# LeonardoTemperanza/LupinPathTracer

Measured on AMD Instinct MI355X. Metric: Msamples/sec (paths x bounces), higher is better.
Workload: dtype f32; 1 GPU; bistro_class 3840x2160, 16 bounces, 8 spp per step, Standard integrator, software BVH (BASELINE configs[4] frame; stand-in scene for bistroexterior, SURVEY 8d); frames_in_flight=1, frames_per_wavefront=6, first_pass_stack_entries=26, traversal=binary

## Files before the change

### lupinpathtracer_amd/csrc/lupin_stages.hpp

```cpp
#pragma once

#include <hip/hip_runtime.h>
#include <hip/hip_fp16.h>

#include "lupin_device.hpp"
#include "../../include/lupin_tiles.h"

using namespace lpd;


constexpr uint32_t META_BOUNCE_MASK = 0xFFFu;
constexpr uint32_t META_VOLUME = 1u << 12;
constexpr uint32_t META_NEXT_EMISSION = 1u << 13;
constexpr uint32_t META_TERMINATED = 1u << 14;
constexpr uint32_t META_SAMPLE_SHIFT = 16;
constexpr uint32_t HIT_MISS = 0xFFFFFFFFu;

template <typename T>
struct PathField
{
    char *base;
    uint32_t stride;
    __device__ __forceinline__ T &operator[](size_t slot) const { return *reinterpret_cast<T *>(base + slot * stride); }
};
// ... 97 lines not shown
    ori = mk3(m[0][0] * e.x + m[1][0] * e.y + m[2][0] * e.z + m[3][0] * 1.0f,
              m[0][1] * e.x + m[1][1] * e.y + m[2][1] * e.z + m[3][1] * 1.0f,
              m[0][2] * e.x + m[1][2] * e.y + m[2][2] * e.z + m[3][2] * 1.0f);
    dir = normalize3(mk3(m[0][0] * d.x + m[1][0] * d.y + m[2][0] * d.z + m[3][0] * 0.0f,
                         m[0][1] * d.x + m[1][1] * d.y + m[2][1] * d.z + m[3][1] * 0.0f,
                         m[0][2] * d.x + m[1][2] * d.y + m[2][2] * d.z + m[3][2] * 0.0f));
}

__device__ __forceinline__ void slot_to_pixel(const FrameParams &fp, uint32_t slot, uint32_t &gx, uint32_t &gy)
{
    if (fp.tile_px)
    {
        const uint32_t per_tile = fp.tile_px * fp.tile_px;
        const uint32_t t = lupin_owned_tile(slot / per_tile, fp.rank, fp.world, fp.tiles_x);
        const uint32_t r = slot % per_tile;
        gx = (t % fp.tiles_x) * fp.tile_px + r % fp.tile_px;
        gy = (t / fp.tiles_x) * fp.tile_px + r / fp.tile_px;
        return;
    }
    gx = fp.off_x + slot % fp.reg_w;
    gy = fp.off_y + slot / fp.reg_w;
}

__device__ __forceinline__ void queue_append(bool alive, uint32_t slot, uint32_t *queue, uint32_t *counter)
{
    const unsigned long long mask = __ballot(alive);
    if (mask)
    {
        const int lane = threadIdx.x & 63;
        const int leader = __ffsll((long long)mask) - 1;
        uint32_t base = 0;
        if (lane == leader) base = atomicAdd(counter, (uint32_t)__popcll(mask));
        base = __shfl(base, leader);
        if (alive) queue[base + __popcll(mask & ((1ull << lane) - 1ull))] = slot;
    }
}


__global__ void k_set_params(FrameParams fp, FrameParams *dst) { *dst = fp; }

template <bool ADAPTIVE>
__device__ __forceinline__ void begin_paths(const FrameParams *__restrict__ fpp, PathBuffers pb, uint32_t n,
                                            const uint8_t *__restrict__ block_active, const uint32_t *__restrict__ frames, uint32_t blocks_x)
{
    const FrameParams fp = *fpp;
    uint32_t slot = blockIdx.x * LP_BLOCK + threadIdx.x;
    uint32_t gx = 0, gy = 0, frame = 0;
    bool live = slot < n;
    if (live)
    {
        uint32_t pslot;
        frame = slot_frame(fp, slot, pslot);
        slot_to_pixel(fp, pslot, gx, gy);
        live = gx < fp.width && gy < fp.height;
        if (ADAPTIVE && live) live = block_active[(gy >> 3) * blocks_x + (gx >> 3)] != 0;
    }
    const uint32_t shard = blockIdx.x % LP_SHARDS;
    queue_append(live, slot, pb.queue[0] + (size_t)shard * pb.shard_cap, &pb.counts[shard]);
    if (!live) return;
    const FrameParams &ff = fpp[frame];
    uint32_t counter = ff.pc.accum_counter;
    if (ADAPTIVE) counter += frames[(size_t)gy * fp.width + gx];
    uint32_t rng = rng_seed_for(gy * fp.width + gx, counter);
    f3 o, d;
    camera_ray(ff, gx, gy, rng, o, d);
    pb.ori_rng[slot] = make_float4(o.x, o.y, o.z, __uint_as_float(rng));
    pb.dir_meta[slot] = make_float4(d.x, d.y, d.z, __uint_as_float(META_NEXT_EMISSION));
    pb.weight[slot] = make_float4(1.0f, 1.0f, 1.0f, 0.0f);
    pb.radiance[slot] = make_float4(0.0f, 0.0f, 0.0f, 0.0f);
    pb.color[slot] = make_float4(0.0f, 0.0f, 0.0f, 0.0f);
    pb.next_hit[slot] = make_float4(0.0f, 0.0f, 0.0f, __uint_as_float(HIT_MISS));
    pb.next_tri[slot] = 0u;
}

__global__ void __launch_bounds__(LP_BLOCK) k_begin(const FrameParams *__restrict__ fpp, PathBuffers pb, uint32_t n)
{
    begin_paths<false>(fpp, pb, n, nullptr, nullptr, 0u);
}

#ifndef LP_EXTEND_WAVES
#define LP_EXTEND_WAVES 4
#endif
#ifndef LP_SHADE_WAVES
#define LP_SHADE_WAVES 3
#endif
#ifndef LP_DEFER_SHADE_WAVES
#define LP_DEFER_SHADE_WAVES 4
#endif
#ifndef LP_LIGHT_PDF_WAVES
#define LP_LIGHT_PDF_WAVES 4
#endif
#ifndef LP_LIGHT_PDF_MIS_WAVES
#define LP_LIGHT_PDF_MIS_WAVES 3
#endif
#ifndef LP_MIS_DEFER_SHADE_WAVES
#define LP_MIS_DEFER_SHADE_WAVES 3
#endif
#ifndef LP_SIMPLE_SHADE_WAVES
#define LP_SIMPLE_SHADE_WAVES 4
#endif
#ifndef LP_MIS_SHADE_WAVES
#define LP_MIS_SHADE_WAVES 2
#endif
template <bool LDSGEO> struct GeoOf { typedef GeoGlobal type; };
template <> struct GeoOf<true> { typedef GeoLds type; };
template <bool LDSGEO>
__device__ __forceinline__ typename GeoOf<LDSGEO>::type make_geo(const SceneDev &sc, uint32_t *lds, uint32_t stack_words);
template <>
__device__ __forceinline__ GeoGlobal make_geo<false>(const SceneDev &sc, uint32_t *, uint32_t) { return geo_global(sc); }
template <>
__device__ __forceinline__ GeoLds make_geo<true>(const SceneDev &sc, uint32_t *lds, uint32_t stack_words)
{
    GeoLds g = geo_stage_lds(sc, lds + stack_words);
    __syncthreads();
    return g;
}

template <typename Geo, bool OPAQUE = false>
__device__ __forceinline__ void trace_alpha(const Geo &geo, const SceneDev &sc, uint32_t *stack, f3 o, f3 d, uint32_t &rng, float eps,
                                            float4 &hitrec, uint32_t &hit_tri)
{
    float total = 0.0f;
    Closest c;
    c.t = LP_F32_MAX; c.u = 0.0f; c.v = 0.0f; c.tri = 0u; c.inst = HIT_MISS;
    bool hit = false;
    for (uint32_t k = 0; k < 128u; k++)
    {
        c = scene_closest(geo, sc, stack, o, d, eps);
        hit = (c.t != LP_F32_MAX);
        if (!hit) break;
        total += c.t;
        if (OPAQUE || !(sc.instances[c.inst].flags & 1u)) break;
        Surface s = resolve_surface(sc, c.inst, c.tri, c.u, c.v);
        float opacity = surface_opacity(sc, s);
        if (opacity < 1.0f && rnd(rng) >= opacity) o = add(o, scale(d, c.t));
        else break;
    }
    hitrec = make_float4(total, c.u, c.v, __uint_as_float(hit ? c.inst : HIT_MISS));
    hit_tri = c.tri;
}

constexpr int LP_TALLY = 4;
constexpr int LP_ROUND_BASE = 12, LP_ROUND_WORDS = 10;
constexpr int LP_CLOCK_BASE = 22, LP_CLOCK_WORDS = 6;
__device__ __forceinline__ void tally_flush(const uint32_t (&tally)[LP_TALLY], unsigned long long *work)
{
    #pragma unroll
    for (int k = 0; k < LP_TALLY; k++)
    {
        uint32_t v = tally[k];
        #pragma unroll
        for (int off = 32; off > 0; off >>= 1) v += __shfl_xor(v, off);
        if ((threadIdx.x & 63u) == 0u && v) atomicAdd(&work[k], (unsigned long long)v);
    }
}
template <typename Geo, bool COUNT> struct TallyOf { typedef Geo type; };
template <typename Geo> struct TallyOf<Geo, true> { typedef GeoTally<Geo> type; };
template <bool COUNT, typename Geo>
__device__ __forceinline__ typename TallyOf<Geo, COUNT>::type with_tally(const Geo &geo, uint32_t *tally)
{
    if constexpr (COUNT) { GeoTally<Geo> g; g.base = geo; g.tally = tally; return g; }
    else return geo;
}

template <int TYPE, bool LDSGEO, bool OPAQUE, bool COUNT>
__global__ void __attribute__((amdgpu_waves_per_eu(LP_EXTEND_WAVES, 8))) __launch_bounds__(LP_BLOCK) k_extend(SceneDev sc, const FrameParams *__restrict__ fpp, PathBuffers pb, uint32_t iter,
                                                     unsigned long long *shard_stats, uint32_t stack_words, unsigned long long *work)
// ... 399 lines not shown
    const auto geo = geo_global(sc);
    for (uint32_t k = 0; k < (MODE == 1 ? 2u : 1u); k++)
    {
        bool have = i < count;
        f3 o = splat(0.0f), d = mk3(0.0f, 0.0f, 1.0f);
        if (have)
        {
            const uint32_t slot = pb.queue[iter & 1][(size_t)shard * pb.shard_cap + i];
            if (MODE == 0)
            {
                const float4 orr = pb.ori_rng[slot], dm = pb.dir_meta[slot];
                o = mk3(orr.x, orr.y, orr.z); d = mk3(dm.x, dm.y, dm.z);
            }
            else
            {
                const float4 so = pb.sh_org[slot];
                have = (__float_as_uint(so.w) & (1u << k)) != 0;
                const float4 dd = k ? pb.sh_d1[slot] : pb.sh_d0[slot];
                o = mk3(so.x, so.y, so.z); d = mk3(dd.x, dd.y, dd.z);
            }
        }
        if (have)
        {
            const Closest a = scene_closest(geo, sc, lds_stack, o, d, eps);
            bool flag;
            uint32_t why = 0u;
            const Closest b = scene_closest_wide(geo, sc, lds_stack, wide_pairs, o, d, eps, flag, &why);
            why_tie += (why & WIDE_WHY_TIE) ? 1u : 0u; why_cond += (why & WIDE_WHY_CONDITION) ? 1u : 0u;
            why_leaky += (why & WIDE_WHY_LEAKY) ? 1u : 0u; why_stack += (why & WIDE_WHY_STACK) ? 1u : 0u;
            const bool miss_a = a.t == LP_F32_MAX, miss_b = b.t == LP_F32_MAX;
            const bool same = (miss_a && miss_b) || (!miss_a && !miss_b && __float_as_uint(a.t) == __float_as_uint(b.t) && __float_as_uint(a.u) == __float_as_uint(b.u) &&
                                                     __float_as_uint(a.v) == __float_as_uint(b.v) && a.tri == b.tri && a.inst == b.inst);
            checked += 1u; flagged += flag ? 1u : 0u; raw += same ? 0u : 1u; bad += (!same && !flag) ? 1u : 0u;
            if (!same && !flag)
                printf("[lupin verify] uncertified difference: mode %d o %a %a %a d %a %a %a | binary t %a tri %u inst %u | wide t %a tri %u inst %u\n", MODE,
                       o.x, o.y, o.z, d.x, d.y, d.z, a.t, a.tri, a.inst, b.t, b.tri, b.inst);
        }
    }
    uint32_t v[8] = {checked, flagged, bad, raw, why_tie, why_cond, why_leaky, why_stack};
    #pragma unroll
    for (int k = 0; k < 8; k++)
    {
        uint32_t x = v[k];
        #pragma unroll
        for (int off = 32; off > 0; off >>= 1) x += __shfl_xor(x, off);
        if ((threadIdx.x & 63u) == 0u && x) atomicAdd(&verify[k], (unsigned long long)x);
    }
}

__device__ __forceinline__ f3 clamp_radiance(f3 r, float max_radiance)
{
    if (!finite3(r)) r = splat(0.0f);
    if (r.x > max_radiance || r.y > max_radiance || r.z > max_radiance)
        r = scale(r, max_radiance / maxf(r.x, maxf(r.y, r.z)));
    return r;
}

struct ShadowRays
{
    PathBuffers *pb;
    uint32_t slot;
    uint32_t flags;
    __device__ __forceinline__ void emit(int k, f3 org, f3 dir, f3 factor, float scalar)
    {
        flags |= 1u << k;
        if (!pb) return;
        pb->sh_org[slot] = make_float4(org.x, org.y, org.z, 0.0f);
        if (k == 0) { pb->sh_d0[slot] = make_float4(dir.x, dir.y, dir.z, scalar); pb->sh_f0[slot] = make_float4(factor.x, factor.y, factor.z, 0.0f); }
        else        { pb->sh_d1[slot] = make_float4(dir.x, dir.y, dir.z, scalar); pb->sh_f1[slot] = make_float4(factor.x, factor.y, factor.z, 0.0f); }
    }
};

struct PathRegs
{
    f3 ori, dir, weight, radiance;
    uint32_t rng;
    int bounce;
    bool in_medium;
    bool next_emission;
    Medium medium;
    bool pending;
    f3 pend_f;
    float pend_bp;
};

__device__ __forceinline__ bool weight_checks_and_roulette(PathRegs &p)
{
    if (is_zero3(p.weight) || !finite3(p.weight)) return false;
    if (p.bounce > 3)
    {
        float survive = minf(0.99f, maxf(p.weight.x, maxf(p.weight.y, p.weight.z)));
        if (rnd(p.rng) >= survive) return false;
        p.weight = scale(p.weight, 1.0f / survive);
    }
    return true;
}

template <int TYPE, typename Geo, bool SIMPLE = false, bool DEFER = false>
__device__ __forceinline__ bool integrate_vertex(const Geo &geo, const SceneDev &sc, uint32_t *stack, const FrameParams &fp, PathRegs &p,
                                 float4 hitrec, uint32_t hit_tri, ShadowRays &sh)
{
    static_assert(!DEFER || TYPE == LUPIN_PATHTRACE_STANDARD || TYPE == LUPIN_PATHTRACE_MIS, "the light-pdf stage serves the Standard and MIS integrators");
    constexpr bool DEFER_WEIGHT = DEFER && TYPE == LUPIN_PATHTRACE_STANDARD;
    const float eps = fp.pc.ray_epsilon;
    const uint32_t hit_inst = __float_as_uint(hitrec.w);
    p.pending = false;
    if (hit_inst == HIT_MISS)
    {
        if (TYPE != LUPIN_PATHTRACE_DIRECT || p.next_emission)
            p.radiance = add(p.radiance, mul(p.weight, environment_radiance(sc, p.dir)));
        return false;
    }
    const float hit_dst = hitrec.x;

    bool in_volume = false;
    float volume_dst = hit_dst;
    if (p.in_medium)
    {
        float r1 = rnd(p.rng);
        float r2 = rnd(p.rng);
        volume_dst = medium_sample_distance(p.medium.density, hit_dst, r1, r2);
        f3 tr = medium_transmittance(p.medium.density, volume_dst);
        float tp = medium_distance_pdf(p.medium.density, volume_dst, hit_dst);
        p.weight = mul(p.weight, divs(tr, tp));
        in_volume = volume_dst < hit_dst;
    }

    const f3 outgoing = neg(p.dir);
    f3 incoming = splat(0.0f);
    f3 hit_pos;
    if (!in_volume)
    {
        hit_pos = add(p.ori, scale(p.dir, hit_dst));
        const Surface s = resolve_surface(sc, hit_inst, hit_tri, hitrec.y, hitrec.z);
        const MatPoint mp = material_point<SIMPLE>(sc, s);
        const f3 normal = shading_normal(geo, sc, s);

        if (TYPE == LUPIN_PATHTRACE_STANDARD || TYPE == LUPIN_PATHTRACE_NAIVE || p.next_emission)
            p.radiance = add(p.radiance, mul(p.weight, mp.emission));

        const bool delta = mat_is_delta(mp);

        if (TYPE == LUPIN_PATHTRACE_DIRECT)
        {
            if (!delta)
            {
                f3 li = lights_sample(sc, hit_pos, p.rng);
                float pdf = lights_pdf(geo, sc, stack, hit_pos, li, eps);
                f3 bsdfcos = bsdf_eval(mp, normal, outgoing, li);
                if (none_zero3(bsdfcos) && pdf > 0.0f)
                {
                    sh.emit(1, hit_pos, li, mul(p.weight, bsdfcos), pdf);
                }
                p.next_emission = false;
            }
            else p.next_emission = true;
        }

        if (!delta)
        {
            if (TYPE == LUPIN_PATHTRACE_STANDARD || TYPE == LUPIN_PATHTRACE_DIRECT)
            {
                if (rnd(p.rng) < 0.5f)
                {
                    float rnl = rnd(p.rng);
                    float ra = rnd(p.rng), rb = rnd(p.rng);
                    incoming = bsdf_sample(mp, normal, outgoing, rnl, ra, rb);
                }
                else incoming = lights_sample(sc, hit_pos, p.rng);
                if (is_zero3(incoming)) return false;
                if (DEFER_WEIGHT)
                {
                    p.pend_bp = bsdf_pdf(mp, normal, outgoing, incoming);
                    p.pend_f = bsdf_eval(mp, normal, outgoing, incoming);
                    p.pending = true;
                }
                else
                {
                    float prob = 0.5f * bsdf_pdf(mp, normal, outgoing, incoming) + 0.5f * lights_pdf(geo, sc, stack, hit_pos, incoming, eps);
                    p.weight = mul(p.weight, divs(bsdf_eval(mp, normal, outgoing, incoming), prob));
                }
            }
            else if (TYPE == LUPIN_PATHTRACE_NAIVE)
            {
                float rnl = rnd(p.rng);
                float ra = rnd(p.rng), rb = rnd(p.rng);
                incoming = bsdf_sample(mp, normal, outgoing, rnl, ra, rb);
                if (is_zero3(incoming)) return false;
                p.weight = mul(p.weight, divs(bsdf_eval(mp, normal, outgoing, incoming), bsdf_pdf(mp, normal, outgoing, incoming)));
            }
            else
            {
                f3 bsdfcos0 = splat(0.0f);
                float b_pdf0 = 0.0f;
                bool have0 = false;
                #pragma unroll(DEFER ? 2 : 1)
                for (int k = 0; k < 2; k++)
                {
                    const bool light_turn = (k != 0);
                    f3 normal_k = normal, outgoing_k = outgoing;
                    MatPoint mp_k = mp;
                    asm volatile("" : "+v"(normal_k.x), "+v"(normal_k.y), "+v"(normal_k.z), "+v"(outgoing_k.x), "+v"(outgoing_k.y), "+v"(outgoing_k.z),
                                      "+v"(mp_k.color.x), "+v"(mp_k.color.y), "+v"(mp_k.color.z), "+v"(mp_k.roughness), "+v"(mp_k.metallic), "+v"(mp_k.ior));
                    f3 mi;
                    if (light_turn) mi = lights_sample(sc, hit_pos, p.rng);
                    else
                    {
                        float rnl = rnd(p.rng);
                        float ra = rnd(p.rng), rb = rnd(p.rng);
                        mi = bsdf_sample(mp_k, normal_k, outgoing_k, rnl, ra, rb);
                    }
                    if (is_zero3(mi)) break;
                    if (!light_turn) incoming = mi;

                    if (DEFER)
                    {
                        const f3 bsdfcos = bsdf_eval(mp_k, normal_k, outgoing_k, mi);
                        const float bp = bsdf_pdf(mp_k, normal_k, outgoing_k, mi);
                        if (!light_turn) { bsdfcos0 = bsdfcos; b_pdf0 = bp; have0 = true; }
                        if (none_zero3(bsdfcos)) sh.emit(k, hit_pos, mi, mul(p.weight, bsdfcos), bp);
                        continue;
                    }
                    const float light_pdf = lights_pdf(geo, sc, stack, hit_pos, mi, eps);
                    const f3 bsdfcos = bsdf_eval(mp_k, normal_k, outgoing_k, mi);
                    const float b_pdf = bsdf_pdf(mp_k, normal_k, outgoing_k, mi);
                    if (!light_turn) { bsdfcos0 = bsdfcos; b_pdf0 = b_pdf; have0 = true; }
                    float mis_w;
                    if (light_turn) mis_w = (light_pdf * light_pdf) / (light_pdf * light_pdf + b_pdf * b_pdf) / light_pdf;
                    else            mis_w = (b_pdf * b_pdf) / (b_pdf * b_pdf + light_pdf * light_pdf) / b_pdf;

                    if (none_zero3(bsdfcos) && mis_w != 0.0f) sh.emit(k, hit_pos, mi, mul(p.weight, bsdfcos), mis_w);
                }
                if (have0) p.weight = mul(p.weight, divs(bsdfcos0, b_pdf0));
                else p.weight = mul(p.weight, divs(bsdf_eval(mp, normal, outgoing, incoming), bsdf_pdf(mp, normal, outgoing, incoming)));
                p.next_emission = false;
            }
        }
        else
        {
            incoming = delta_sample(mp, normal, outgoing, rnd(p.rng));
            if (is_zero3(incoming)) return false;
            p.weight = mul(p.weight, divs(delta_eval(mp, normal, outgoing, incoming), delta_pdf(mp, normal, outgoing, incoming)));
            if (TYPE == LUPIN_PATHTRACE_MIS) p.next_emission = true;
        }

        if (mat_is_volumetric(mp) && dot3(normal, outgoing) * dot3(normal, incoming) < 0.0f)
        {
            if (!p.in_medium)
            {
                p.medium.density = mp.density;
                p.medium.scattering = mp.scattering;
                p.medium.anisotropy = mp.anisotropy;
                p.in_medium = true;
            }
            else p.in_medium = false;
        }
    }
    else
    {
        hit_pos = add(p.ori, scale(p.dir, volume_dst));
        if (TYPE == LUPIN_PATHTRACE_NAIVE)
        {
            float unused0 = rnd(p.rng); (void)unused0;
            float ra = rnd(p.rng), rb = rnd(p.rng);
            incoming = phase_sample(p.medium, outgoing, ra, rb);
            if (is_zero3(incoming)) return false;
            float prob = phase_pdf(p.medium, outgoing, incoming);
            p.weight = mul(p.weight, divs(phase_eval(p.medium, outgoing, incoming), prob));
        }
        else
        {
            if (rnd(p.rng) < 0.5f)
            {
                float unused0 = rnd(p.rng); (void)unused0;
                float ra = rnd(p.rng), rb = rnd(p.rng);
                incoming = phase_sample(p.medium, outgoing, ra, rb);
            }
            else incoming = lights_sample(sc, hit_pos, p.rng);
            if (TYPE == LUPIN_PATHTRACE_MIS) p.next_emission = true;
            if (is_zero3(incoming)) return false;
            if (DEFER_WEIGHT)
            {
                p.pend_bp = phase_pdf(p.medium, outgoing, incoming);
                p.pend_f = phase_eval(p.medium, outgoing, incoming);
                p.pending = true;
            }
            else
            {
                float prob = 0.5f * phase_pdf(p.medium, outgoing, incoming) + 0.5f * lights_pdf(geo, sc, stack, hit_pos, incoming, eps);
                p.weight = mul(p.weight, divs(phase_eval(p.medium, outgoing, incoming), prob));
            }
        }
    }

    p.ori = hit_pos;
    p.dir = incoming;
    if (DEFER_WEIGHT && p.pending) return true;
    return weight_checks_and_roulette(p);
}

template <int TYPE>
__device__ __forceinline__ bool path_epilogue(const FrameParams &fp, const FrameParams *fpp, PathBuffers &pb, uint32_t slot, PathRegs &p, uint32_t sample, bool cont,
                                              bool vol_dirty, float4 r4)
{
    bool alive = false;
    if (cont)
    {
        alive = true;
        if (vol_dirty)
        {
            pb.vol0[slot] = make_float4(p.medium.density.x, p.medium.density.y, p.medium.density.z, p.medium.anisotropy);
            pb.vol1[slot] = make_float4(p.medium.scattering.x, p.medium.scattering.y, p.medium.scattering.z, 0.0f);
        }
        pb.weight[slot] = make_float4(p.weight.x, p.weight.y, p.weight.z, 0.0f);
        if (p.radiance.x != r4.x || p.radiance.y != r4.y || p.radiance.z != r4.z)
            pb.radiance[slot] = make_float4(p.radiance.x, p.radiance.y, p.radiance.z, 0.0f);
    }
    else
    {
        float4 c4 = pb.color[slot];
        f3 cr = clamp_radiance(p.radiance, fp.pc.max_radiance);
        pb.color[slot] = make_float4(c4.x + cr.x, c4.y + cr.y, c4.z + cr.z, 0.0f);
        sample++;
        if (sample < fp.spp)
        {
            alive = true;
            uint32_t gx, gy, pslot;
            const uint32_t frame = slot_frame(fp, slot, pslot);
            slot_to_pixel(fp, pslot, gx, gy);
            camera_ray(fpp[frame], gx, gy, p.rng, p.ori, p.dir);
            p.bounce = 0;
            p.in_medium = false;
            p.next_emission = true;
            pb.weight[slot] = make_float4(1.0f, 1.0f, 1.0f, 0.0f);
            pb.radiance[slot] = make_float4(0.0f, 0.0f, 0.0f, 0.0f);
            if (TYPE == LUPIN_PATHTRACE_MIS)
            {
                pb.next_hit[slot] = make_float4(0.0f, 0.0f, 0.0f, __uint_as_float(HIT_MISS));
                pb.next_tri[slot] = 0u;
            }
        }
    }
    if (alive)
    {
        uint32_t nm = ((uint32_t)p.bounce & META_BOUNCE_MASK) | (p.in_medium ? META_VOLUME : 0u) |
                      (p.next_emission ? META_NEXT_EMISSION : 0u) | (sample << META_SAMPLE_SHIFT);
        pb.ori_rng[slot] = make_float4(p.ori.x, p.ori.y, p.ori.z, __uint_as_float(p.rng));
        pb.dir_meta[slot] = make_float4(p.dir.x, p.dir.y, p.dir.z, __uint_as_float(nm));
    }
    return alive;
}

enum : int { SLOT_DONE = 0, SLOT_ALIVE = 1, SLOT_WAITS_FOR_LIGHT_PDF = 2 };
constexpr uint32_t QUEUE_STATE_SHIFT = 30u, QUEUE_SLOT_MASK = (1u << QUEUE_STATE_SHIFT) - 1u, QUEUE_ENTRY_NONE = 0xFFFFFFFFu;

template <int TYPE, typename Geo, bool SIMPLE = false, bool DEFER = false>
__device__ __forceinline__ int shade_path(const Geo &geo, const SceneDev &sc, uint32_t *stack, const FrameParams &fp, const FrameParams *fpp, PathBuffers &pb,
                                          uint32_t slot, float4 orr, float4 dm, uint32_t rng, float4 hitrec, uint32_t hit_tri)
{
    float4 w4 = pb.weight[slot];
    float4 r4 = pb.radiance[slot];
    uint32_t meta = __float_as_uint(dm.w);

    PathRegs p;
    p.ori = mk3(orr.x, orr.y, orr.z);
    p.dir = mk3(dm.x, dm.y, dm.z);
    p.weight = mk3(w4.x, w4.y, w4.z);
    p.radiance = mk3(r4.x, r4.y, r4.z);
    p.rng = rng;
    p.bounce = (int)(meta & META_BOUNCE_MASK);
    p.in_medium = SIMPLE ? false : (meta & META_VOLUME) != 0;
    p.next_emission = (meta & META_NEXT_EMISSION) != 0;
    uint32_t sample = meta >> META_SAMPLE_SHIFT;
    const bool was_in_medium = p.in_medium;
    if (p.in_medium)
    {
        float4 a = pb.vol0[slot], b = pb.vol1[slot];
        p.medium.density = mk3(a.x, a.y, a.z);
        p.medium.anisotropy = a.w;
        p.medium.scattering = mk3(b.x, b.y, b.z);
    }
    else { p.medium.density = splat(0.0f); p.medium.scattering = splat(0.0f); p.medium.anisotropy = 0.0f; }

    ShadowRays sh;
    sh.pb = (TYPE == LUPIN_PATHTRACE_MIS || TYPE == LUPIN_PATHTRACE_DIRECT) ? &pb : nullptr;
    sh.slot = slot;
    sh.flags = 0u;
    bool cont = integrate_vertex<TYPE, Geo, SIMPLE, DEFER>(geo, sc, stack, fp, p, hitrec, hit_tri, sh);
    const bool vol_dirty = p.in_medium && !was_in_medium;
    if (DEFER && cont && p.pending)
    {
        if (vol_dirty)
        {
            pb.vol0[slot] = make_float4(p.medium.density.x, p.medium.density.y, p.medium.density.z, p.medium.anisotropy);
            pb.vol1[slot] = make_float4(p.medium.scattering.x, p.medium.scattering.y, p.medium.scattering.z, 0.0f);
        }
        if (was_in_medium) pb.weight[slot] = make_float4(p.weight.x, p.weight.y, p.weight.z, 0.0f);
        if (p.radiance.x != r4.x || p.radiance.y != r4.y || p.radiance.z != r4.z)
            pb.radiance[slot] = make_float4(p.radiance.x, p.radiance.y, p.radiance.z, 0.0f);
        pb.sh_f0[slot] = make_float4(p.pend_f.x, p.pend_f.y, p.pend_f.z, p.pend_bp);
        const uint32_t nm = ((uint32_t)p.bounce & META_BOUNCE_MASK) | (p.in_medium ? META_VOLUME : 0u) |
                            (p.next_emission ? META_NEXT_EMISSION : 0u) | (sample << META_SAMPLE_SHIFT);
        pb.ori_rng[slot] = make_float4(p.ori.x, p.ori.y, p.ori.z, __uint_as_float(p.rng));
        pb.dir_meta[slot] = make_float4(p.dir.x, p.dir.y, p.dir.z, __uint_as_float(nm));
        return SLOT_WAITS_FOR_LIGHT_PDF;
    }
    if (cont)
    {
        p.bounce++;
        if (p.bounce > (int)fp.max_bounces) cont = false;
    }

    if (TYPE == LUPIN_PATHTRACE_MIS || TYPE == LUPIN_PATHTRACE_DIRECT)
    {
        if (vol_dirty)
        {
            pb.vol0[slot] = make_float4(p.medium.density.x, p.medium.density.y, p.medium.density.z, p.medium.anisotropy);
            pb.vol1[slot] = make_float4(p.medium.scattering.x, p.medium.scattering.y, p.medium.scattering.z, 0.0f);
        }
        pb.weight[slot] = make_float4(p.weight.x, p.weight.y, p.weight.z, 0.0f);
        pb.radiance[slot] = make_float4(p.radiance.x, p.radiance.y, p.radiance.z, 0.0f);
        const uint32_t nm = ((uint32_t)p.bounce & META_BOUNCE_MASK) | (p.in_medium ? META_VOLUME : 0u) |
                            (p.next_emission ? META_NEXT_EMISSION : 0u) | (cont ? 0u : META_TERMINATED) | (sample << META_SAMPLE_SHIFT);
        pb.ori_rng[slot] = make_float4(p.ori.x, p.ori.y, p.ori.z, __uint_as_float(p.rng));
        pb.dir_meta[slot] = make_float4(p.dir.x, p.dir.y, p.dir.z, __uint_as_float(nm));
        pb.sh_org[slot].w = __uint_as_float(sh.flags);
        return SLOT_ALIVE;
    }
    return path_epilogue<TYPE>(fp, fpp, pb, slot, p, sample, cont, vol_dirty, r4) ? SLOT_ALIVE : SLOT_DONE;
}

template <int TYPE, typename Geo>
__device__ __forceinline__ bool light_pdf_path(const Geo &geo, const SceneDev &sc, uint32_t *stack, const FrameParams &fp, const FrameParams *fpp, PathBuffers &pb, uint32_t slot)
{
    const float4 orr = pb.ori_rng[slot], dm = pb.dir_meta[slot], w4 = pb.weight[slot], pd = pb.sh_f0[slot];
    const uint32_t meta = __float_as_uint(dm.w);
    PathRegs p;
    p.ori = mk3(orr.x, orr.y, orr.z);
    p.dir = mk3(dm.x, dm.y, dm.z);
    p.weight = mk3(w4.x, w4.y, w4.z);
    p.rng = __float_as_uint(orr.w);
    p.bounce = (int)(meta & META_BOUNCE_MASK);
    p.in_medium = (meta & META_VOLUME) != 0;
    p.next_emission = (meta & META_NEXT_EMISSION) != 0;
    p.pending = false;
    const uint32_t sample = meta >> META_SAMPLE_SHIFT;

    const float prob = 0.5f * pd.w + 0.5f * lights_pdf(geo, sc, stack, p.ori, p.dir, fp.pc.ray_epsilon);
    p.weight = mul(p.weight, divs(mk3(pd.x, pd.y, pd.z), prob));
    bool cont = weight_checks_and_roulette(p);
    if (cont)
    {
        p.bounce++;
        if (p.bounce > (int)fp.max_bounces) cont = false;
    }
    float4 r4 = make_float4(0.0f, 0.0f, 0.0f, 0.0f);
    if (!cont) r4 = pb.radiance[slot];
    p.radiance = mk3(r4.x, r4.y, r4.z);
    return path_epilogue<TYPE>(fp, fpp, pb, slot, p, sample, cont, false, r4);
}

#ifndef LP_SORT_WINDOW
#define LP_SORT_WINDOW 4096
#endif
template <bool PEEK_COIN, bool FROM_TRACER>
__global__ void __launch_bounds__(LP_BLOCK) k_sort_queue(SceneDev sc, PathBuffers pb, uint32_t iter, uint32_t in_place)
{
    constexpr uint32_t PER_THREAD = LP_SORT_WINDOW / LP_BLOCK;
    constexpr uint32_t NUM_KEYS = LP_SORT_KEYS;
    __shared__ uint32_t sorted[LP_SORT_WINDOW];
    __shared__ uint32_t bins[NUM_KEYS];
    const uint32_t shard = blockIdx.x % LP_SHARDS;
    const uint32_t count = pb.counts[iter * LP_SHARDS + shard];
    const uint32_t base_i = (blockIdx.x / LP_SHARDS) * LP_SORT_WINDOW;
    if (base_i >= count) return;
    uint32_t *entries = pb.queue[iter & 1] + (size_t)shard * pb.shard_cap + base_i;
    uint32_t *order = in_place ? entries : pb.shade_order + (size_t)shard * pb.shard_cap + base_i;
    const uint32_t valid = min(LP_SORT_WINDOW, count - base_i);
    if (threadIdx.x < NUM_KEYS) bins[threadIdx.x] = 0u;
    __syncthreads();
    uint32_t my_slot[PER_THREAD], my_key[PER_THREAD], my_rank[PER_THREAD];
    #pragma unroll
    for (uint32_t r = 0; r < PER_THREAD; r++) my_slot[r] = entries[min(r * LP_BLOCK + threadIdx.x, valid - 1u)];
    if constexpr (FROM_TRACER)
    {
        #pragma unroll
        for (uint32_t r = 0; r < PER_THREAD; r++) my_key[r] = pb.skey[my_slot[r]] & (NUM_KEYS - 1u);
    }
    else
    {
        uint32_t hit_w[PER_THREAD], meta_w[PER_THREAD], rng_w[PER_THREAD], flags_w[PER_THREAD];
        #pragma unroll
        for (uint32_t r = 0; r < PER_THREAD; r++)
        {
            hit_w[r] = __float_as_uint(pb.hit[my_slot[r]].w);
            meta_w[r] = __float_as_uint(pb.dir_meta[my_slot[r]].w);
            rng_w[r] = PEEK_COIN ? __float_as_uint(pb.ori_rng[my_slot[r]].w) : 0u;
        }
        #pragma unroll
        for (uint32_t r = 0; r < PER_THREAD; r++) flags_w[r] = sc.instances[hit_w[r] == HIT_MISS ? 0u : hit_w[r]].flags;
        #pragma unroll
        for (uint32_t r = 0; r < PER_THREAD; r++) my_key[r] = shade_sort_key<PEEK_COIN>((meta_w[r] & META_VOLUME) != 0, hit_w[r] == HIT_MISS, flags_w[r], rng_w[r]);
    }
    #pragma unroll
    for (uint32_t r = 0; r < PER_THREAD; r++)
    {
        my_rank[r] = 0u;
        if (r * LP_BLOCK + threadIdx.x < valid) my_rank[r] = atomicAdd(&bins[my_key[r]], 1u);
    }
    __syncthreads();
    if (threadIdx.x < 64)
    {
        const uint32_t c = bins[threadIdx.x];
        uint32_t incl = c;
        for (int off = 1; off < 64; off <<= 1) { const uint32_t v = (uint32_t)__shfl_up((int)incl, off); if ((int)threadIdx.x >= off) incl += v; }
        bins[threadIdx.x] = incl - c;
    }
    __syncthreads();
    #pragma unroll
    for (uint32_t r = 0; r < PER_THREAD; r++)
        if (r * LP_BLOCK + threadIdx.x < valid) sorted[bins[my_key[r]] + my_rank[r]] = in_place ? my_slot[r] : base_i + r * LP_BLOCK + threadIdx.x;
    __syncthreads();
    #pragma unroll
    for (uint32_t r = 0; r < PER_THREAD; r++)
    {
        const uint32_t j = r * LP_BLOCK + threadIdx.x;
        if (j < valid) order[j] = sorted[j];
    }
}

__global__ void __launch_bounds__(LP_BLOCK) k_compact_queue(PathBuffers pb, uint32_t iter)
{
    constexpr uint32_t PER_THREAD = LP_SORT_WINDOW / LP_BLOCK;
    static_assert(PER_THREAD % 4 == 0, "a thread reads its entries as uint4");
    __shared__ uint32_t wave_total[LP_BLOCK / 64];
    __shared__ uint32_t window_base;
    const uint32_t shard = blockIdx.x % LP_SHARDS;
    const uint32_t count = pb.counts[iter * LP_SHARDS + shard];
    const uint32_t base_i = (blockIdx.x / LP_SHARDS) * LP_SORT_WINDOW;
    if (base_i >= count) return;
    const uint32_t valid = min(LP_SORT_WINDOW, count - base_i);
    const uint32_t *entries = pb.queue[iter & 1] + (size_t)shard * pb.shard_cap + base_i;
    const uint32_t first = threadIdx.x * PER_THREAD;
    uint32_t e[PER_THREAD];
    if (first + PER_THREAD <= valid)
    {
        #pragma unroll
        for (uint32_t r = 0; r < PER_THREAD / 4; r++)
        {
            const uint4 v = reinterpret_cast<const uint4 *>(entries + first)[r];
            e[4 * r] = v.x; e[4 * r + 1] = v.y; e[4 * r + 2] = v.z; e[4 * r + 3] = v.w;
        }
    }
    else
    {
        #pragma unroll
        for (uint32_t r = 0; r < PER_THREAD; r++) e[r] = first + r < valid ? entries[first + r] : QUEUE_ENTRY_NONE;
    }
    uint32_t mine = 0;
    #pragma unroll
    for (uint32_t r = 0; r < PER_THREAD; r++) mine += e[r] != QUEUE_ENTRY_NONE ? 1u : 0u;
    const uint32_t wave = threadIdx.x >> 6, lane = threadIdx.x & 63;
    uint32_t incl = mine;
    for (int off = 1; off < 64; off <<= 1) { const uint32_t v = (uint32_t)__shfl_up((int)incl, off); if ((int)lane >= off) incl += v; }
    if (lane == 63) wave_total[wave] = incl;
    __syncthreads();
    uint32_t before = incl - mine, total = 0;
    for (uint32_t w = 0; w < LP_BLOCK / 64; w++) { const uint32_t c = wave_total[w]; if (w < wave) before += c; total += c; }
    if (total == 0) return;
    if (threadIdx.x == 0) window_base = atomicAdd(&pb.counts[(iter + 1) * LP_SHARDS + shard], total);
    __syncthreads();
    uint32_t *out = pb.queue[(iter + 1) & 1] + (size_t)shard * pb.shard_cap + window_base + before;
    #pragma unroll
    for (uint32_t r = 0; r < PER_THREAD; r++)
        if (e[r] != QUEUE_ENTRY_NONE) *out++ = e[r];
}

template <int TYPE, bool LDSGEO, bool SIMPLE, bool DEFER = false>
__global__ void __attribute__((amdgpu_waves_per_eu(TYPE == 1 ? (DEFER ? LP_MIS_DEFER_SHADE_WAVES : LP_MIS_SHADE_WAVES) : (SIMPLE ? LP_SIMPLE_SHADE_WAVES : (DEFER ? LP_DEFER_SHADE_WAVES : LP_SHADE_WAVES)), 8))) __launch_bounds__(LP_BLOCK) k_shade(SceneDev sc, const FrameParams *__restrict__ fpp, PathBuffers pb, uint32_t iter,
                                                    unsigned long long *shard_stats, uint32_t stack_words)
{
    const FrameParams fp = *fpp;
    if (SIMPLE) sc.num_envs = 0;
    extern __shared__ __attribute__((aligned(16))) uint32_t lds_stack[];
    const auto geo = make_geo<LDSGEO>(sc, lds_stack, stack_words);
    const uint32_t shard = blockIdx.x % LP_SHARDS;
    const uint32_t count = pb.counts[iter * LP_SHARDS + shard];
    const uint32_t i = (blockIdx.x / LP_SHARDS) * LP_BLOCK + threadIdx.x;
    constexpr bool PERMUTED = TYPE != LUPIN_PATHTRACE_MIS && TYPE != LUPIN_PATHTRACE_DIRECT;
    uint32_t *const entries = pb.queue[iter & 1] + (size_t)shard * pb.shard_cap;
    int state = SLOT_DONE;
    bool mine = i < count;
    uint32_t slot = 0, pos = i;
    if (PERMUTED && mine && sc.sort_shade) pos = pb.shade_order[(size_t)shard * pb.shard_cap + i];
    if (mine) slot = entries[pos];
    if (mine)
    {
        const float4 orr = pb.ori_rng[slot];
        state = shade_path<TYPE, typename GeoOf<LDSGEO>::type, SIMPLE, DEFER>(geo, sc, lds_stack, fp, fpp, pb, slot, orr, pb.dir_meta[slot], __float_as_uint(orr.w), pb.hit[slot], pb.hit_tri[slot]);
    }
    if (i == 0 && iter == 0) shard_stats[shard * 2 + 1] += (unsigned long long)count * fp.spp;
    if (TYPE == LUPIN_PATHTRACE_MIS || TYPE == LUPIN_PATHTRACE_DIRECT) return;
    if (!SIMPLE && mine && sc.sort_shade) pos = pb.shade_order[(size_t)shard * pb.shard_cap + i];
    if (DEFER)
    {
        if (mine) entries[pos] = slot | ((uint32_t)state << QUEUE_STATE_SHIFT);
        return;
    }
    if (sc.sort_shade)
    {
        if (mine) entries[pos] = state == SLOT_ALIVE ? slot : QUEUE_ENTRY_NONE;
        return;
    }
    queue_append(state == SLOT_ALIVE, slot, pb.queue[(iter + 1) & 1] + (size_t)shard * pb.shard_cap, &pb.counts[(iter + 1) * LP_SHARDS + shard]);
}

template <int TYPE, bool LDSGEO>
__global__ void __attribute__((amdgpu_waves_per_eu(LP_LIGHT_PDF_WAVES, 8))) __launch_bounds__(LP_BLOCK) k_light_pdf(SceneDev sc, const FrameParams *__restrict__ fpp, PathBuffers pb, uint32_t iter, uint32_t stack_words)
{
    const FrameParams fp = *fpp;
    extern __shared__ __attribute__((aligned(16))) uint32_t lds_stack[];
    __shared__ uint32_t waiting[LP_BLOCK];
    __shared__ uint32_t entry_slot[LP_BLOCK];
    __shared__ uint32_t verdict[LP_BLOCK];
    __shared__ uint32_t wave_total[LP_BLOCK / 64];
    const auto geo = make_geo<LDSGEO>(sc, lds_stack, stack_words);
    const uint32_t shard = blockIdx.x % LP_SHARDS;
    const uint32_t count = pb.counts[iter * LP_SHARDS + shard];
    const uint32_t i = (blockIdx.x / LP_SHARDS) * LP_BLOCK + threadIdx.x;
    if ((blockIdx.x / LP_SHARDS) * LP_BLOCK >= count) return;
    uint32_t *entries = pb.queue[iter & 1] + (size_t)shard * pb.shard_cap + (size_t)(blockIdx.x / LP_SHARDS) * LP_BLOCK;
    const uint32_t entry = i < count ? entries[threadIdx.x] : QUEUE_ENTRY_NONE;
    const uint32_t state = entry == QUEUE_ENTRY_NONE ? (uint32_t)SLOT_DONE : entry >> QUEUE_STATE_SHIFT;
    const uint32_t slot = entry & QUEUE_SLOT_MASK;
    const bool waits = state == (uint32_t)SLOT_WAITS_FOR_LIGHT_PDF;
    const unsigned long long wmask = __ballot(waits);
    const uint32_t wave = threadIdx.x >> 6, lane = threadIdx.x & 63;
    if (lane == 0) wave_total[wave] = (uint32_t)__popcll(wmask);
    verdict[threadIdx.x] = 0u;
    entry_slot[threadIdx.x] = slot;
    __syncthreads();
    uint32_t before = 0, total = 0;
    for (uint32_t w = 0; w < LP_BLOCK / 64; w++) { const uint32_t c = wave_total[w]; if (w < wave) before += c; total += c; }
    if (waits) waiting[before + (uint32_t)__popcll(wmask & ((1ull << lane) - 1ull))] = threadIdx.x;
    __syncthreads();
    if (threadIdx.x < total)
    {
        const uint32_t w = waiting[threadIdx.x];
        if (light_pdf_path<TYPE, typename GeoOf<LDSGEO>::type>(geo, sc, lds_stack, fp, fpp, pb, entry_slot[w])) verdict[w] = 1u;
    }
    __syncthreads();
    const bool alive = state == (uint32_t)SLOT_ALIVE || (waits && verdict[threadIdx.x] != 0u);
    queue_append(alive, slot, pb.queue[(iter + 1) & 1] + (size_t)shard * pb.shard_cap, &pb.counts[(iter + 1) * LP_SHARDS + shard]);
}

template <bool LDSGEO>
__global__ void __attribute__((amdgpu_waves_per_eu(LP_LIGHT_PDF_MIS_WAVES, 8))) __launch_bounds__(LP_BLOCK) k_light_pdf_mis(SceneDev sc, const FrameParams *__restrict__ fpp, PathBuffers pb, uint32_t iter, uint32_t stack_words)
{
    const FrameParams fp = *fpp;
    extern __shared__ __attribute__((aligned(16))) uint32_t lds_stack[];
    __shared__ uint32_t items[2 * LP_BLOCK];
    __shared__ uint32_t entry_slot[LP_BLOCK], entry_flags[LP_BLOCK];
// ... 700 lines not shown
```

Measured before the change: 1605 Msamples/s.

## Cut live registers across light-pdf BVH march in Standard shade kernel

Restructures the Standard integrator's vertex update so the BSDF/phase pdf and eval are computed and pinned before the lights_pdf BVH traversal. The volume-stack update and its buffer write now happen before the march, and radiance dirtiness is tracked as a flag rather than by comparing against a saved float4. This shrinks the live state held across the traversal, and the Standard shade kernel's waves-per-EU target is raised from 3 to 4, with a separate knob for the Direct integrator. The risks are spills or a worse schedule from the asm pins, plus extra stores of volume state.

```diff
diff --git a/lupinpathtracer_amd/csrc/lupin_stages.hpp b/lupinpathtracer_amd/csrc/lupin_stages.hpp
--- a/lupinpathtracer_amd/csrc/lupin_stages.hpp
+++ b/lupinpathtracer_amd/csrc/lupin_stages.hpp
@@ -203,7 +203,10 @@
 #define LP_EXTEND_WAVES 4
 #endif
 #ifndef LP_SHADE_WAVES
-#define LP_SHADE_WAVES 3
+#define LP_SHADE_WAVES 4
+#endif
+#ifndef LP_DIRECT_SHADE_WAVES
+#define LP_DIRECT_SHADE_WAVES 3
 #endif
 #ifndef LP_DEFER_SHADE_WAVES
 #define LP_DEFER_SHADE_WAVES 4
@@ -769,6 +772,7 @@
     bool pending;
     f3 pend_f;
     float pend_bp;
+    bool radiance_dirty;
 };
 
 __device__ __forceinline__ bool weight_checks_and_roulette(PathRegs &p)
@@ -783,15 +787,41 @@
     return true;
 }
 
+__device__ __forceinline__ void update_volume_stack(PathRegs &p, const MatPoint &mp, f3 normal, f3 outgoing, f3 incoming, PathBuffers *vol_pb, uint32_t vol_slot)
+{
+    if (mat_is_volumetric(mp) && dot3(normal, outgoing) * dot3(normal, incoming) < 0.0f)
+    {
+        if (!p.in_medium)
+        {
+            p.medium.density = mp.density;
+            p.medium.scattering = mp.scattering;
+            p.medium.anisotropy = mp.anisotropy;
+            p.in_medium = true;
+            if (vol_pb)
+            {
+                vol_pb->vol0[vol_slot] = make_float4(mp.density.x, mp.density.y, mp.density.z, mp.anisotropy);
+                vol_pb->vol1[vol_slot] = make_float4(mp.scattering.x, mp.scattering.y, mp.scattering.z, 0.0f);
+            }
+        }
+        else p.in_medium = false;
+    }
+}
+
+__device__ __forceinline__ void pin_before_march(f3 &f, float &bp)
+{
+    asm volatile("" : "+v"(f.x), "+v"(f.y), "+v"(f.z), "+v"(bp));
+}
+
 template <int TYPE, typename Geo, bool SIMPLE = false, bool DEFER = false>
 __device__ __forceinline__ bool integrate_vertex(const Geo &geo, const SceneDev &sc, uint32_t *stack, const FrameParams &fp, PathRegs &p,
-                                 float4 hitrec, uint32_t hit_tri, ShadowRays &sh)
+                                 float4 hitrec, uint32_t hit_tri, ShadowRays &sh, PathBuffers *vol_pb = nullptr, uint32_t vol_slot = 0u)
 {
     static_assert(!DEFER || TYPE == LUPIN_PATHTRACE_STANDARD || TYPE == LUPIN_PATHTRACE_MIS, "the light-pdf stage serves the Standard and MIS integrators");
     constexpr bool DEFER_WEIGHT = DEFER && TYPE == LUPIN_PATHTRACE_STANDARD;
     const float eps = fp.pc.ray_epsilon;
     const uint32_t hit_inst = __float_as_uint(hitrec.w);
     p.pending = false;
+    p.radiance_dirty = false;
     if (hit_inst == HIT_MISS)
     {
         if (TYPE != LUPIN_PATHTRACE_DIRECT || p.next_emission)
@@ -816,6 +846,9 @@
     const f3 outgoing = neg(p.dir);
     f3 incoming = splat(0.0f);
     f3 hit_pos;
+    bool march = false;
+    f3 march_f = splat(0.0f);
+    float march_bp = 0.0f;
     if (!in_volume)
     {
         hit_pos = add(p.ori, scale(p.dir, hit_dst));
@@ -824,17 +857,24 @@
         const f3 normal = shading_normal(geo, sc, s);
 
         if (TYPE == LUPIN_PATHTRACE_STANDARD || TYPE == LUPIN_PATHTRACE_NAIVE || p.next_emission)
+        {
+            const f3 before = p.radiance;
             p.radiance = add(p.radiance, mul(p.weight, mp.emission));
+            p.radiance_dirty = p.radiance.x != before.x || p.radiance.y != before.y || p.radiance.z != before.z;
+        }
 
         const bool delta = mat_is_delta(mp);
+        bool volume_done = false;
 
         if (TYPE == LUPIN_PATHTRACE_DIRECT)
         {
             if (!delta)
             {
                 f3 li = lights_sample(sc, hit_pos, p.rng);
+                f3 bsdfcos;
+                if (!SIMPLE) bsdfcos = bsdf_eval(mp, normal, outgoing, li);
                 float pdf = lights_pdf(geo, sc, stack, hit_pos, li, eps);
-                f3 bsdfcos = bsdf_eval(mp, normal, outgoing, li);
+                if (SIMPLE) bsdfcos = bsdf_eval(mp, normal, outgoing, li);
                 if (none_zero3(bsdfcos) && pdf > 0.0f)
                 {
                     sh.emit(1, hit_pos, li, mul(p.weight, bsdfcos), pdf);
@@ -864,8 +904,11 @@
                 }
                 else
                 {
-                    float prob = 0.5f * bsdf_pdf(mp, normal, outgoing, incoming) + 0.5f * lights_pdf(geo, sc, stack, hit_pos, incoming, eps);
-                    p.weight = mul(p.weight, divs(bsdf_eval(mp, normal, outgoing, incoming), prob));
+                    march_bp = bsdf_pdf(mp, normal, outgoing, incoming);
+                    march_f = bsdf_eval(mp, normal, outgoing, incoming);
+                    update_volume_stack(p, mp, normal, outgoing, incoming, vol_pb, vol_slot);
+                    volume_done = true;
+                    march = true;
                 }
             }
             else if (TYPE == LUPIN_PATHTRACE_NAIVE)
@@ -931,17 +974,7 @@
             if (TYPE == LUPIN_PATHTRACE_MIS) p.next_emission = true;
         }
 
-        if (mat_is_volumetric(mp) && dot3(normal, outgoing) * dot3(normal, incoming) < 0.0f)
-        {
-            if (!p.in_medium)
-            {
-                p.medium.density = mp.density;
-                p.medium.scattering = mp.scattering;
-                p.medium.anisotropy = mp.anisotropy;
-                p.in_medium = true;
-            }
-            else p.in_medium = false;
-        }
+        if (!volume_done) update_volume_stack(p, mp, normal, outgoing, incoming, vol_pb, vol_slot);
     }
     else
     {
@@ -972,12 +1005,25 @@
                 p.pend_f = phase_eval(p.medium, outgoing, incoming);
                 p.pending = true;
             }
-            else
+            else if (TYPE == LUPIN_PATHTRACE_MIS)
             {
                 float prob = 0.5f * phase_pdf(p.medium, outgoing, incoming) + 0.5f * lights_pdf(geo, sc, stack, hit_pos, incoming, eps);
                 p.weight = mul(p.weight, divs(phase_eval(p.medium, outgoing, incoming), prob));
             }
-        }
+            else
+            {
+                march_bp = phase_pdf(p.medium, outgoing, incoming);
+                march_f = phase_eval(p.medium, outgoing, incoming);
+                march = true;
+            }
+        }
+    }
+
+    if (march)
+    {
+        pin_before_march(march_f, march_bp);
+        float prob = 0.5f * march_bp + 0.5f * lights_pdf(geo, sc, stack, hit_pos, incoming, eps);
+        p.weight = mul(p.weight, divs(march_f, prob));
     }
 
     p.ori = hit_pos;
@@ -988,7 +1034,7 @@
 
 template <int TYPE>
 __device__ __forceinline__ bool path_epilogue(const FrameParams &fp, const FrameParams *fpp, PathBuffers &pb, uint32_t slot, PathRegs &p, uint32_t sample, bool cont,
-                                              bool vol_dirty, float4 r4)
+                                              bool vol_dirty, bool radiance_dirty)
 {
     bool alive = false;
     if (cont)
@@ -1000,7 +1046,7 @@
             pb.vol1[slot] = make_float4(p.medium.scattering.x, p.medium.scattering.y, p.medium.scattering.z, 0.0f);
         }
         pb.weight[slot] = make_float4(p.weight.x, p.weight.y, p.weight.z, 0.0f);
-        if (p.radiance.x != r4.x || p.radiance.y != r4.y || p.radiance.z != r4.z)
+        if (radiance_dirty)
             pb.radiance[slot] = make_float4(p.radiance.x, p.radiance.y, p.radiance.z, 0.0f);
     }
     else
@@ -1073,8 +1119,10 @@
     sh.pb = (TYPE == LUPIN_PATHTRACE_MIS || TYPE == LUPIN_PATHTRACE_DIRECT) ? &pb : nullptr;
     sh.slot = slot;
     sh.flags = 0u;
-    bool cont = integrate_vertex<TYPE, Geo, SIMPLE, DEFER>(geo, sc, stack, fp, p, hitrec, hit_tri, sh);
-    const bool vol_dirty = p.in_medium && !was_in_medium;
+    constexpr bool EARLY_VOL = !DEFER && (TYPE == LUPIN_PATHTRACE_STANDARD || TYPE == LUPIN_PATHTRACE_DIRECT);
+    bool cont = integrate_vertex<TYPE, Geo, SIMPLE, DEFER>(geo, sc, stack, fp, p, hitrec, hit_tri, sh, EARLY_VOL ? &pb : nullptr, slot);
+    if (EARLY_VOL) asm volatile("" : "+v"(slot));
+    const bool vol_dirty = !EARLY_VOL && p.in_medium && !was_in_medium;
     if (DEFER && cont && p.pending)
     {
         if (vol_dirty)
@@ -1083,7 +1131,7 @@
             pb.vol1[slot] = make_float4(p.medium.scattering.x, p.medium.scattering.y, p.medium.scattering.z, 0.0f);
         }
         if (was_in_medium) pb.weight[slot] = make_float4(p.weight.x, p.weight.y, p.weight.z, 0.0f);
-        if (p.radiance.x != r4.x || p.radiance.y != r4.y || p.radiance.z != r4.z)
+        if (p.radiance_dirty)
             pb.radiance[slot] = make_float4(p.radiance.x, p.radiance.y, p.radiance.z, 0.0f);
         pb.sh_f0[slot] = make_float4(p.pend_f.x, p.pend_f.y, p.pend_f.z, p.pend_bp);
         const uint32_t nm = ((uint32_t)p.bounce & META_BOUNCE_MASK) | (p.in_medium ? META_VOLUME : 0u) |
@@ -1114,7 +1162,7 @@
         pb.sh_org[slot].w = __uint_as_float(sh.flags);
         return SLOT_ALIVE;
     }
-    return path_epilogue<TYPE>(fp, fpp, pb, slot, p, sample, cont, vol_dirty, r4) ? SLOT_ALIVE : SLOT_DONE;
+    return path_epilogue<TYPE>(fp, fpp, pb, slot, p, sample, cont, vol_dirty, p.radiance_dirty) ? SLOT_ALIVE : SLOT_DONE;
 }
 
 template <int TYPE, typename Geo>
@@ -1144,7 +1192,7 @@
     float4 r4 = make_float4(0.0f, 0.0f, 0.0f, 0.0f);
     if (!cont) r4 = pb.radiance[slot];
     p.radiance = mk3(r4.x, r4.y, r4.z);
-    return path_epilogue<TYPE>(fp, fpp, pb, slot, p, sample, cont, false, r4);
+    return path_epilogue<TYPE>(fp, fpp, pb, slot, p, sample, cont, false, p.radiance.x != r4.x || p.radiance.y != r4.y || p.radiance.z != r4.z);
 }
 
 #ifndef LP_SORT_WINDOW
@@ -1264,7 +1312,7 @@
 }
 
 template <int TYPE, bool LDSGEO, bool SIMPLE, bool DEFER = false>
-__global__ void __attribute__((amdgpu_waves_per_eu(TYPE == 1 ? (DEFER ? LP_MIS_DEFER_SHADE_WAVES : LP_MIS_SHADE_WAVES) : (SIMPLE ? LP_SIMPLE_SHADE_WAVES : (DEFER ? LP_DEFER_SHADE_WAVES : LP_SHADE_WAVES)), 8))) __launch_bounds__(LP_BLOCK) k_shade(SceneDev sc, const FrameParams *__restrict__ fpp, PathBuffers pb, uint32_t iter,
+__global__ void __attribute__((amdgpu_waves_per_eu(TYPE == 1 ? (DEFER ? LP_MIS_DEFER_SHADE_WAVES : LP_MIS_SHADE_WAVES) : (SIMPLE ? LP_SIMPLE_SHADE_WAVES : (DEFER ? LP_DEFER_SHADE_WAVES : (TYPE == 3 ? LP_DIRECT_SHADE_WAVES : LP_SHADE_WAVES))), 8))) __launch_bounds__(LP_BLOCK) k_shade(SceneDev sc, const FrameParams *__restrict__ fpp, PathBuffers pb, uint32_t iter,
                                                     unsigned long long *shard_stats, uint32_t stack_words)
 {
     const FrameParams fp = *fpp;
```

New measurement: 1638 Msamples/s (median of 6 runs). 1.02x the previous value.
